# BradenDKelly/MetropolisMonteCarlo

Measured on AMD Instinct MI355X. Metric: MC trial moves/sec (whole node), SPC/E NVT full Ewald fp64, higher is better.
Workload: dtype f64

## Files before the change

metropolismontecarlo_amd/csrc/mmc_wave.hpp:

```cpp
#pragma once
#include "mmc_fast.hpp"
#include "mmc_propose.hpp"

#ifndef WV_WAVES
#define WV_WAVES 4
#endif
#ifndef WV_OCC
#define WV_OCC 5
#endif
#ifndef WV_OCC_WOLF
#define WV_OCC_WOLF 4
#endif
#ifndef WV_MWAVES
#define WV_MWAVES WV_WAVES
#endif
#ifndef WV_LIST
#define WV_LIST 640
#endif
#ifndef WV_PF
#define WV_PF 6
#endif
#define MMC_CQ_PAD (4 * 64 * (2 * WV_PF + 2))
#ifndef WV_TPF
#define WV_TPF 3
// ... 39 lines not shown
    __builtin_amdgcn_fence(__ATOMIC_ACQUIRE, "wavefront");
}

__device__ __forceinline__ double dpp_quad_swap_f64(double v)
{
    const long long b = __double_as_longlong(v);
    const unsigned lo = (unsigned)__builtin_amdgcn_update_dpp(0, (int)b, 0xB1, 0xf, 0xf, true),
                   hi = (unsigned)__builtin_amdgcn_update_dpp(0, (int)(b >> 32), 0xB1, 0xf, 0xf, true);
    return __longlong_as_double((long long)(((unsigned long long)hi << 32) | lo));
}
__device__ __forceinline__ void wave_sum6_add(double v0, double v1, double v2, double v3, double v4,
                                              double v5, double *out, double *scratch, int lane)
{
    const bool odd = (lane & 1) != 0;
    double p0 = (odd ? v1 : v0) + dpp_quad_swap_f64(odd ? v0 : v1);
    double p1 = (odd ? v3 : v2) + dpp_quad_swap_f64(odd ? v2 : v3);
    double p2 = (odd ? v5 : v4) + dpp_quad_swap_f64(odd ? v4 : v5);
    p0 += dpp_row_shr_f64<2>(p0); p1 += dpp_row_shr_f64<2>(p1); p2 += dpp_row_shr_f64<2>(p2);
    p0 += dpp_row_shr_f64<4>(p0); p1 += dpp_row_shr_f64<4>(p1); p2 += dpp_row_shr_f64<4>(p2);
    p0 += dpp_row_shr_f64<8>(p0); p1 += dpp_row_shr_f64<8>(p1); p2 += dpp_row_shr_f64<8>(p2);
    if ((lane & 14) == 14) {
        double *dst = scratch + 4 * (lane & 1) + (lane >> 4);
        dst[0] = p0; dst[8] = p1; dst[16] = p2;
    }
    __builtin_amdgcn_fence(__ATOMIC_RELEASE, "wavefront");
    __builtin_amdgcn_wave_barrier();
    __builtin_amdgcn_fence(__ATOMIC_ACQUIRE, "wavefront");
    if (lane < 6) {
        const double *r = scratch + 4 * lane;
        out[lane] += ((r[0] + r[1]) + r[2]) + r[3];
    }
}
__device__ __forceinline__ void wave_sum4_add(double v0, double v1, double v4, double v5, double *out,
                                              double *scratch, int lane)
{
    const bool odd = (lane & 1) != 0;
    double p0 = (odd ? v1 : v0) + dpp_quad_swap_f64(odd ? v0 : v1);
    double p1 = (odd ? v5 : v4) + dpp_quad_swap_f64(odd ? v4 : v5);
    p0 += dpp_row_shr_f64<2>(p0); p1 += dpp_row_shr_f64<2>(p1);
    p0 += dpp_row_shr_f64<4>(p0); p1 += dpp_row_shr_f64<4>(p1);
    p0 += dpp_row_shr_f64<8>(p0); p1 += dpp_row_shr_f64<8>(p1);
    if ((lane & 14) == 14) {
        double *dst = scratch + 4 * (lane & 1) + (lane >> 4);
        dst[0] = p0; dst[8] = p1;
    }
    __builtin_amdgcn_fence(__ATOMIC_RELEASE, "wavefront");
    __builtin_amdgcn_wave_barrier();
    __builtin_amdgcn_fence(__ATOMIC_ACQUIRE, "wavefront");
    if (lane < 4) {
        const double *r = scratch + 4 * lane;
        out[lane < 2 ? lane : lane + 2] += ((r[0] + r[1]) + r[2]) + r[3];
    }
}
__device__ __forceinline__ void wave_sum1_store(double v, double *out, double *scratch, int lane)
{
    v += dpp_row_shr_f64<1>(v);
    v += dpp_row_shr_f64<2>(v);
    v += dpp_row_shr_f64<4>(v);
    v += dpp_row_shr_f64<8>(v);
    if ((lane & 15) == 15)
        scratch[lane >> 4] = v;
    __builtin_amdgcn_fence(__ATOMIC_RELEASE, "wavefront");
    __builtin_amdgcn_wave_barrier();
    __builtin_amdgcn_fence(__ATOMIC_ACQUIRE, "wavefront");
    if (lane == 0)
        *out = ((scratch[0] + scratch[1]) + scratch[2]) + scratch[3];
}

__device__ __forceinline__ int lane_i32(int v, int src)
{
    return __builtin_amdgcn_readlane(v, src);
}

__device__ __forceinline__ double uniform_f64(double v)
{
    const long long b = __double_as_longlong(v);
    unsigned lo, hi;
    asm volatile("v_readfirstlane_b32 %0, %1" : "=s"(lo) : "v"((int)b));
    asm volatile("v_readfirstlane_b32 %0, %1" : "=s"(hi) : "v"((int)(b >> 32)));
    return __longlong_as_double((long long)(((unsigned long long)hi << 32) | lo));
}

__device__ __forceinline__ double lane_f64(double v, int src)
{
    const long long b = __double_as_longlong(v);
    const unsigned lo = (unsigned)__builtin_amdgcn_readlane((int)b, src);
    const unsigned hi = (unsigned)__builtin_amdgcn_readlane((int)(b >> 32), src);
    return __longlong_as_double((long long)(((unsigned long long)hi << 32) | lo));
}

__device__ __forceinline__ unsigned long long wave_shfl_xor_u64(unsigned long long v, int m)
{
    const unsigned lo = (unsigned)__shfl_xor((int)(unsigned)v, m, 64);
    const unsigned hi = (unsigned)__shfl_xor((int)(unsigned)(v >> 32), m, 64);
    return ((unsigned long long)hi << 32) | lo;
}
__device__ __forceinline__ unsigned long long wave_min_u64(unsigned long long v)
{
#pragma unroll
    for (int m = 32; m > 0; m >>= 1) {
        const unsigned long long o = wave_shfl_xor_u64(v, m);
        v = o < v ? o : v;
    }
    return v;
}

__device__ __forceinline__ void phase_row_moderate(double x, double L, cplx *row )
{
    double sn, cs;
    sincos_moderate(MMC_TWOPI * x / L, sn, cs);
    const cplx e1 = { cs, sn }, one = { 1.0, 0.0 };
    row[5] = one;
    row[6] = e1;
    row[4] = c_conj(e1);
    cplx p = e1;
#pragma unroll
    for (int k = 2; k <= 5; k++) {
        p = c_mul(p, e1);
        row[5 + k] = p;
        row[5 - k] = c_conj(p);
    }
}

__device__ __forceinline__ int wave_decide(const double *outw, bool ov_old, bool ov_new,
                                           const DecideConsts *__restrict__ dc, long long step, int r,
                                           int scur, int lane, double *delta_out = nullptr, bool store_flags = true,
                                           bool flip_s = true)
{
    const double delta = mmc_move_delta(outw, ov_old, ov_new, dc->factor);
    if (delta_out)
        *delta_out = delta;
    const double x = delta / dc->temperature;
    const double u = mmc_metropolis_uniform(ChainKey{ dc->seed, dc->replica0 + (uint32_t)r }, (uint64_t)step);
    bool met;
    if (x < 0.0) met = true;
    else if (1.0 - x > u + 1e-9) met = true;
    else if ((1.0 + x) * u > 1.0 + 1e-9) met = false;
    else met = exp(-x) > u;
    const int acc = (met && !(ov_old || ov_new)) ? 1 : 0;
    if (store_flags && lane == 0)
        dc->flags[r] = (uint8_t)(acc | ((scur ^ (flip_s ? acc : 0)) << 1));
    return acc;
}

__device__ __forceinline__ int wave_ticket(unsigned *queue, unsigned base, int n_waves, int lane)
{
    unsigned t = 0;
    if (lane == 0)
        t = atomicAdd(queue, 1u);
    return n_waves + (int)(__builtin_amdgcn_readfirstlane(t) - base);
}

template <bool SUBST, bool IMG, bool MULTI = false, bool WOLF = false>
__global__ __launch_bounds__(WV_MWAVES * 64)
__attribute__((amdgpu_waves_per_eu(WOLF ? WV_OCC_WOLF : WV_OCC, WOLF ? WV_OCC_WOLF : WV_OCC))) void k_move_eval_wave(
    BatchView bv, double *rec, const double *__restrict__ qq_tab,
    const int32_t *__restrict__ kpack, FastConsts fc, const MoveRec *__restrict__ cur,
    const MoveRec *__restrict__ prev, PartOut *out, int n_parts, PairParams pp, int r_base,
    int n_units, const uint8_t *flagv, unsigned stamp, const DecideConsts *__restrict__ dc, long long dec_step,
    int n_sub_arg, int slot0, unsigned *queue, unsigned queue_base)
{
    const int n_sub = MULTI ? n_sub_arg : 1;
    __shared__ __align__(16) WaveSharedT<WV_MWAVES, !WOLF> sm;
    const int tid = threadIdx.x, lane0 = tid & 63;
    const int wv = __builtin_amdgcn_readfirstlane(tid >> 6);

    for (int k = tid; k < MMC_QQ_TABLE_DOUBLES; k += WV_MWAVES * 64)
        sm.qtab[k] = qq_tab[k];
    __syncthreads();

    const int n_mol = bv.n_mol, nkv = bv.nkvecs;
    const double box = bv.box;
    const BoxConsts bc = box_consts(box);
    const int np = WOLF ? n_parts : (n_parts == 1) ? 1 : n_parts - 1;
    const int plen = (n_mol + np - 1) / np;
    const bool same_gate = pp.lj_gate_sq == pp.qq_gate_sq;
    const double inv_box = uniform_f64(1.0 / box);
    uint32_t gate_q;
    asm volatile("v_readfirstlane_b32 %0, %1" : "=s"(gate_q) : "v"(com_quant_gate(fmax(pp.lj_gate_sq, pp.qq_gate_sq), box)));
    wv_list_t *const list = sm.list[wv];
    const double *const pvw = sm.pvw[wv];

    for (int unit = blockIdx.x * WV_MWAVES + wv; unit < n_units;
         unit = MULTI && queue ? wave_ticket(queue, queue_base, gridDim.x * WV_MWAVES, lane0)
                               : unit + gridDim.x * WV_MWAVES) {
        int lane = lane0;
        if (!MULTI)
            asm volatile("" : "+v"(lane));
        int rl = unit, part = 0;
        if (n_parts != 1) {
            rl = unit / n_parts;
            part = unit - rl * n_parts;
        }
        const int r = r_base + rl;
        const bool do_pairs = WOLF ? true : (n_parts == 1) || (part < n_parts - 1);
        const bool do_recip = WOLF ? false : (n_parts == 1) || (part == n_parts - 1);
        const int j_begin = do_pairs ? min(part * plen, n_mol) : 0;
        const int j_end = do_pairs ? min(j_begin + plen, n_mol) : 0;
        double *const myrec = rec + (int64_t)r * n_mol * MMC_RSTRIDE;

        int flags_carry = -1;
        double e_sum = 0.0;
        unsigned acc_mask = 0, ovl_mask = 0, kind_mask = 0;
      for (int sub = 0; sub < n_sub; sub++) {
        if (MULTI) {
            lane = lane0;
            asm volatile("" : "+v"(lane));
        }
        const MoveRec *cur_s = cur, *prev_s = prev;
        if (n_sub > 1) {
            const int sl = (slot0 + sub) % dc->ring_slots, slp = (slot0 + sub + dc->ring_slots - 1) % dc->ring_slots;
            cur_s = dc->ring + (int64_t)sl * dc->ring_stride;
            if (sub > 0)
                prev_s = dc->ring + (int64_t)slp * dc->ring_stride;
        }
        WV_STAMP(0);
        const double *mvp = reinterpret_cast<const double *>(cur_s + r);
        double w = 0.0;
        if (lane < MV_Q_NEW)
            w = mvp[lane];
        WV_STAMP(1);
        const int gflag = flags_carry >= 0 ? flags_carry : (flagv ? __builtin_amdgcn_readfirstlane((int)flagv[r]) : -1);
        const long long hdr = __double_as_longlong(w);
        const int i0 = lane_i32((int)hdr, 0) - 1;
        const int flags = gflag >= 0 ? gflag : lane_i32((int)(hdr >> 32), 0);
        const bool commit = prev_s && (flags & 1);
        const int scur = (flags >> 1) & 1;

        int pend = -1;
        if (commit) {
            const double *pvp = reinterpret_cast<const double *>(prev_s + r);
            double pw = 0.0;
            if (lane < 9) pw = pvp[MV_AT_NEW + lane];
            else if (lane < 12) pw = pvp[MV_COM_NEW + lane - 9];
            else if (lane == 12) pw = pvp[0];
            else if (lane < 17) pw = pvp[MV_Q_NEW + lane - 13];
            pend = lane_i32((int)__double_as_longlong(pw), 12) - 1;
            if (lane < 12)
                sm.pvw[wv][lane] = pw;
            if (part == 0 && lane < 12) {
                myrec[(int64_t)pend * MMC_RSTRIDE + lane] = pw;
                if (lane < 9) {
                    const int a = lane / 3, d = lane % 3;
                    (d == 0 ? bv.ax : d == 1 ? bv.ay : bv.az)[r * bv.atom_stride + 3 * pend + a] = pw;
                } else {
                    const int d = lane - 9;
                    (d == 0 ? bv.comx : d == 1 ? bv.comy : bv.comz)[r * bv.mol_stride + pend] = pw;
                    comq_store(bv, r, pend, d, pw, inv_box);
                }
            }
            if (bv.quat) {
                const double q0 = wave_pick(pw, 13), q1 = wave_pick(pw, 14),
                             q2 = wave_pick(pw, 15), q3 = wave_pick(pw, 16);
                if (part == 0 && lane >= 13 && lane < 17)
                    quat_commit(bv, r, pend, lane - 13, pw, q0 * q0 + q1 * q1 + q2 * q2 + q3 * q3 > 0.25);
            }
            wave_sync();
            if (WOLF && !SUBST)
                asm volatile("s_waitcnt vmcnt(0)" ::: "memory");
        }

#define WV_CQ_BASE (bv.comq + (int64_t)r * 3 * bv.cq_stride)
#define WV_PART_DST (out + (int64_t)r * n_parts + part)
        auto decide_here = [&](bool o0, bool o1) -> int {
            if (!dc)
                return 0;
            if (n_sub <= 1)
                return wave_decide(sm.outw[wv], o0, o1, dc, dec_step, r, scur, lane, nullptr, true, !WOLF);
            double delta;
            const bool last = sub + 1 == n_sub;
            const int acc = wave_decide(sm.outw[wv], o0, o1, dc, dec_step + sub, r, scur, lane, &delta, last, !WOLF);
            if (acc) {
                e_sum += delta;
                acc_mask |= 1u << sub;
            }
            if (o0 || o1)
                ovl_mask |= 1u << sub;
            kind_mask |= (unsigned)((lane_i32((int)(hdr >> 32), 0) >> 8) & 1) << sub;
            flags_carry = acc | ((scur ^ (WOLF ? 0 : acc)) << 1);
            if (last) {
                wave_sync();
                if (lane < 7)
                    sm.outw[wv][lane] = lane == 0 ? e_sum
                                 : lane == 1 ? __longlong_as_double((long long)acc_mask | ((long long)ovl_mask << 32))
                                 : lane == 2 ? __longlong_as_double((long long)kind_mask) : 0.0;
                wave_sync();
            }
            return acc;
        };
#define WV_DECIDE(o0, o1) decide_here(o0, o1)
#define WV_RECORD_OVL(o) (n_sub > 1 ? false : (o))
#define WV_STORE_IF (sub + 1 == n_sub)
#define WV_STORE_SYSTEM MULTI
#define WV_ZERO opaque_f64(0.0)
#define WV_SUBST SUBST
#define WV_IMG IMG
#define WV_WOLF WOLF
#define WV_VIRIAL (!MULTI)
#ifndef WV_XY_MOVE
#define WV_XY_MOVE 1
#endif
#define WV_XY WV_XY_MOVE
#define WV_PASSES 2
#define WV_AFTER_PHASE_TABLES                                                                    \
    if (!SUBST && commit)                                                                        \
        asm volatile("s_waitcnt vmcnt(0)" ::: "memory");
#include "mmc_wave_unit.inc"
#undef WV_AFTER_PHASE_TABLES
#undef WV_IMG
#undef WV_WOLF
#undef WV_VIRIAL
#undef WV_PASSES
#undef WV_XY
#undef WV_SUBST
#undef WV_ZERO
#undef WV_CQ_BASE
#undef WV_PART_DST
#undef WV_DECIDE
#undef WV_RECORD_OVL
#undef WV_STORE_IF
#undef WV_STORE_SYSTEM
        if (n_sub > 1)
            asm volatile("s_waitcnt vmcnt(0)" ::: "memory");
      }
    }
}

struct TotalWaveShared {
    alignas(16) double qtab[MMC_QQ_TABLE_DOUBLES];
    int32_t list[WV_WAVES][WV_LIST];
};

#define WV_TOTAL_WAVES_PER_SIMD 5
template <bool COHERENT, bool IMG>
__device__ __forceinline__ void total_wave_body(
    TotalWaveShared &sm, const BatchView &bv, const double *__restrict__ rec,
    const double *__restrict__ qq_tab, const FastConsts &fc, const PairParams &pp, TotalPart *out,
    int units_per_rep, int n_units, int paired, int wg, int n_wgs, int j_chunk = 0)
{
    const int tid = threadIdx.x, lane0 = tid & 63;
    const int wv = __builtin_amdgcn_readfirstlane(tid >> 6);
    for (int k = tid; k < MMC_QQ_TABLE_DOUBLES; k += WV_WAVES * 64)
        sm.qtab[k] = qq_tab[k];
    __syncthreads();

    const int n_mol = bv.n_mol;
    const double box = bv.box;
    const BoxConsts bc = box_consts(box);
    const bool same_gate = pp.lj_gate_sq == pp.qq_gate_sq;
    const double inv_box = 1.0 / box;
    const uint32_t gate_q = com_quant_gate(fmax(pp.lj_gate_sq, pp.qq_gate_sq), box);
    int32_t *const list = sm.list[wv];

    for (int unit = wg * WV_WAVES + wv; unit < n_units; unit += n_wgs * WV_WAVES) {
        int lane = lane0;
        asm volatile("" : "+v"(lane));
        const int r = unit / units_per_rep, u = unit - r * units_per_rep;
        const double *myrec = rec + (int64_t)r * n_mol * MMC_RSTRIDE;
        const uint16_t *cq0 = bv.comq + (int64_t)r * 3 * bv.cq_stride;
        const uint32_t *sxy = reinterpret_cast<const uint32_t *>(cq0);
        const uint16_t *sz = cq0 + 2 * bv.cq_stride;
        double a_lj = 0, a_v = 0, a_q = 0;
        unsigned long long ovm = 0;

        const int n_ch = j_chunk > 0 ? (n_mol + j_chunk - 1) / j_chunk : 1;
        const int j_lo = j_chunk > 0 ? (u % n_ch) * j_chunk : 0;
        const int j_hi = j_chunk > 0 ? min(j_lo + j_chunk, n_mol) : n_mol;
        const int iA = j_chunk > 0 ? u / n_ch : u, iB = n_mol - 1 - u;
        const bool hasB = paired && iB > iA;
        double wAB = 0.0;
        if (lane < MMC_REC)
            wAB = myrec[(int64_t)iA * MMC_RSTRIDE + lane];
        else if (hasB && lane >= 16 && lane < 16 + MMC_REC)
            wAB = myrec[(int64_t)iB * MMC_RSTRIDE + lane - 16];

        auto process = [&](int cnt) {
            wave_sync();
            for (int n0 = 0; n0 < cnt; n0 += 64) {
                const int n = n0 + lane;
                const bool act = n < cnt;
                const int ent = act ? list[n] : 0;
                const int j = ent & ((1 << 27) - 1);
                const bool isB = (ent >> 27) != 0;
                double t[MMC_REC];
                const double2 *src = reinterpret_cast<const double2 *>(myrec + (int64_t)j * MMC_RSTRIDE);
#pragma unroll
                for (int q = 0; q < 6; q++) {
                    const double2 v = src[q];
                    t[2 * q] = v.x;
                    t[2 * q + 1] = v.y;
                }
                const int own0 = isB ? 16 : 0;
                auto mine = [&](int word) { return wave_pick(wAB, own0 + word); };
                const double ccx = mine(9), ccy = mine(10), ccz = mine(11);
                double m[3] = { 0, 0, 0 };
                auto min1 = [&](int d, double a, double b) {
                    if constexpr (IMG)
                        return fma(m[d], bc.neg, b - a);
                    else
                        return vector1D_abs(a, b, bc);
                };
                if constexpr (IMG) {
                    const double dx = t[9] - ccx, dy = t[10] - ccy, dz = t[11] - ccz;
                    m[0] = (fabs(dx) < bc.half) ? 0.0 : copysign(1.0, dx);
                    m[1] = (fabs(dy) < bc.half) ? 0.0 : copysign(1.0, dy);
                    m[2] = (fabs(dz) < bc.half) ? 0.0 : copysign(1.0, dz);
                }
                const double x0 = min1(0, ccx, t[9]), y0 = min1(1, ccy, t[10]), z0 = min1(2, ccz, t[11]);
                const double c0 = x0 * x0 + y0 * y0 + z0 * z0;
                const bool g0 = act && (c0 < pp.qq_gate_sq);
                const bool l0 = same_gate ? g0 : (act && (c0 < pp.lj_gate_sq));
                const unsigned long long gm0 = wave_ballot(g0);
                auto pair_ab = [&](int ab, double ax, double ay, double az, double bx, double by,
                                   double bz) {
                    const double qq = fc.qq9[ab];
                    const bool qneg = (fc.qneg_mask >> ab) & 1;
                    const double px = min1(0, ax, bx), py = min1(1, ay, by), pz = min1(2, az, bz);
                    const double u0 = px * px + py * py + pz * pz;
                    const unsigned long long cm0 = wave_ballot(u0 < pp.ovr) & gm0;
                    const unsigned long long im0 = (IMG ? ~0ULL : wave_ballot(u0 < pp.qq_slack_sq)) & (qneg ? gm0 & ~cm0 : gm0);
                    double e0 = qq_table_eval_lanes(sm.qtab, u0, im0);
                    if (qneg) {
                        ovm |= cm0;
                    } else if (cm0 != 0ULL) {
                        if (((im0 >> lane) & 1) && u0 < MMC_QQ_UMIN) e0 = qq_pair_cold(u0, pp.kappa);
                    }
                    a_q = fma(e0, qq, a_q);
                    const double eps = fc.eps9[ab], sg = fc.sig9[ab];
                    if ((fc.lj_mask >> ab) & 1) {
                        if (l0 && (IMG || u0 < pp.lj_slack_sq)) {
                            const double s2 = sg * sg / u0;
                            const double s6 = s2 * s2 * s2;
                            const double s12 = s6 * s6;
                            const double virab = eps * (2.0 * s12 - s6);
                            const double f0 = (IMG ? px : vector1D(ax, bx, bc)) * virab * s2,
                                         f1 = (IMG ? py : vector1D(ay, by, bc)) * virab * s2,
                                         f2 = (IMG ? pz : vector1D(az, bz, bc)) * virab * s2;
                            a_lj += eps * (s12 - s6);
                            a_v += (IMG ? x0 : vector1D(ccx, t[9], bc)) * f0 + (IMG ? y0 : vector1D(ccy, t[10], bc)) * f1
                                   + (IMG ? z0 : vector1D(ccz, t[11], bc)) * f2;
                        }
                    }
                };
#pragma unroll 1
                for (int a = 0; a < 3; a++) {
                    const double ax = mine(3 * a), ay = mine(3 * a + 1), az = mine(3 * a + 2);
                    pair_ab(3 * a, ax, ay, az, t[0], t[1], t[2]);
                    __builtin_amdgcn_sched_barrier(0);
                    pair_ab(3 * a + 1, ax, ay, az, t[3], t[4], t[5]);
                    __builtin_amdgcn_sched_barrier(0);
                    pair_ab(3 * a + 2, ax, ay, az, t[6], t[7], t[8]);
                    __builtin_amdgcn_sched_barrier(0);
                }
            }
            wave_sync();
        };

        int cnt = 0;
        for (int half = 0; half < (hasB ? 2 : 1); half++) {
            const int i0 = half == 0 ? iA : iB;
            const int woff = half == 0 ? 0 : 16;
            uint32_t cqxy, cqz;
            {
                const int t = lane & 15;
                const int myq = (t >= 9 && t < 12) ? (int)com_quant(wAB, inv_box) : 0;
                cqxy = (uint32_t)lane_i32(myq, woff + 9) | (uint32_t)lane_i32(myq, woff + 10) << 16;
                cqz = (uint32_t)lane_i32(myq, woff + 11);
            }
            const int first = max(i0 + 1, j_lo);
            int base = first & ~63;
            const char *pxy = reinterpret_cast<const char *>(sxy) + 4 * (int64_t)base;
            const char *pz = reinterpret_cast<const char *>(sz) + 2 * (int64_t)base;
            const uint32_t ul4 = 4u * (uint32_t)lane, ul2 = 2u * (uint32_t)lane;
            uint32_t fxy[WV_TPF], fz[WV_TPF];
#pragma unroll
            for (int b = 0; b < WV_TPF; b++) {
                fxy[b] = *reinterpret_cast<const uint32_t *>(pxy + 256 * b + ul4);
                fz[b] = *reinterpret_cast<const uint16_t *>(pz + 128 * b + ul2);
            }
            while (base < j_hi) {
#pragma unroll
                for (int b = 0; b < WV_TPF; b++) {
                    const int j = base + lane;
                    const uint32_t xy = fxy[b], z = fz[b];
                    fxy[b] = *reinterpret_cast<const uint32_t *>(pxy + 256 * (b + WV_TPF) + ul4);
                    fz[b] = *reinterpret_cast<const uint16_t *>(pz + 128 * (b + WV_TPF) + ul2);
                    const bool keep = (com_quant_dist2(xy, z, cqxy, cqz) < gate_q)
                                      && ((uint32_t)(j - first) < (uint32_t)(j_hi - first));
                    const unsigned long long m = wave_ballot(keep);
                    if (keep)
                        list[cnt + lanes_below(m)] = j | (half << 27);
                    cnt += __popcll(m);
                    base += 64;
                }
                pxy += 256 * WV_TPF;
                pz += 128 * WV_TPF;
                if (cnt > WV_LIST - 64 * WV_TPF) {
                    process(cnt);
                    cnt = 0;
                }
            }
        }
        if (cnt)
            process(cnt);
        const double s0 = wave_sum_rows(a_lj), s1 = wave_sum_rows(a_v), s2 = wave_sum_rows(a_q);
        const bool any_ovl = ovm != 0ULL;
        if (lane == 0) {
            TotalPart o;
            o.lj_pot = s0; o.lj_vir = s1; o.qq = s2;
            o.n_ovl = any_ovl ? 1 : 0;
            o._pad = 0;
            if (COHERENT) {
                double *w = reinterpret_cast<double *>(out + unit);
                __hip_atomic_store(w, o.lj_pot, __ATOMIC_RELAXED, __HIP_MEMORY_SCOPE_AGENT);
                __hip_atomic_store(w + 1, o.lj_vir, __ATOMIC_RELAXED, __HIP_MEMORY_SCOPE_AGENT);
                __hip_atomic_store(w + 2, o.qq, __ATOMIC_RELAXED, __HIP_MEMORY_SCOPE_AGENT);
                __hip_atomic_store(reinterpret_cast<long long *>(w + 3), (long long)o.n_ovl,
                                   __ATOMIC_RELAXED, __HIP_MEMORY_SCOPE_AGENT);
            } else {
                out[unit] = o;
            }
        }
    }
}

template <bool IMG>
__global__ __launch_bounds__(WV_WAVES * 64, WV_TOTAL_WAVES_PER_SIMD) void k_total_wave(
    BatchView bv, const double *__restrict__ rec, const double *__restrict__ qq_tab, FastConsts fc,
    PairParams pp, TotalPart *out, int units_per_rep, int n_units, int paired)
{
    __shared__ __align__(16) TotalWaveShared sm;
    total_wave_body<false, IMG>(sm, bv, rec, qq_tab, fc, pp, out, units_per_rep, n_units, paired,
                           (int)blockIdx.x, (int)gridDim.x);
}

__global__ __launch_bounds__(MMC_BLOCK) void k_total_reduce(const TotalPart *parts, int n_parts,
                                                             TotalsRaw *out)
{
    __shared__ double red[4 * MMC_WAVES];
    const int r = blockIdx.x;
    const TotalPart *p = parts + (int64_t)r * n_parts;
    double v[4] = { 0, 0, 0, 0 }, tot[4];
    for (int k = threadIdx.x; k < n_parts; k += MMC_BLOCK) {
        v[0] += p[k].lj_pot; v[1] += p[k].lj_vir; v[2] += p[k].qq; v[3] += (double)p[k].n_ovl;
    }
    block_sum<4>(v, red, tot);
    if (threadIdx.x == 0) {
        TotalsRaw t;
        t.lj_e = 2.0 * (tot[0] * 4);
        t.lj_v = 2.0 * (tot[1] * 24 / 3.0);
        t.qq = 2.0 * tot[2];
        t.n_ovl = tot[3] > 0 ? 1 : 0;
        t._pad = 0;
        out[r] = t;
    }
}

#define SRV_WAVES 8
struct ServerArgs {
    const unsigned long long *ctrl;
    const double2 *steps;
    uint64_t seed, replica0;
    int64_t rng_off;
    int32_t *timeout_flag;
    uint64_t seq_off;
};
#define SRV_ACCEPT 1u
#define SRV_SCUR 2u
#define SRV_STEPS 4u
#define SRV_QUIT 8u
#define SRV_TIMEOUT_TICKS 300000000ULL
#define SRV_GAVE_UP (~0ULL)

__global__ __launch_bounds__(SRV_WAVES * 64, 2) void k_move_server_wave(
    BatchView bv, double *rec, const double *__restrict__ qq_tab,
    const int32_t *__restrict__ kpack, FastConsts fc, PartOut *out, int n_parts, PairParams pp,
    ServerArgs sa)
{
    __shared__ __align__(16) WaveSharedT<SRV_WAVES> sm;
    __shared__ __align__(16) double mvw_all[SRV_WAVES][32];
    __shared__ __align__(16) double comb[8];
    __shared__ unsigned long long ctl;
    const int tid = threadIdx.x;
    int lane = tid & 63;
    const int wv = __builtin_amdgcn_readfirstlane(tid >> 6);
    for (int k = tid; k < MMC_QQ_TABLE_DOUBLES; k += blockDim.x)
        sm.qtab[k] = qq_tab[k];
    __syncthreads();

    const int n_mol = bv.n_mol, nkv = bv.nkvecs;
    const double box = bv.box;
    const BoxConsts bc = box_consts(box);
    const int np = n_parts - 1;
    const int plen = (n_mol + np - 1) / np;
    const bool same_gate = pp.lj_gate_sq == pp.qq_gate_sq;
    const double inv_box = 1.0 / box;
    const uint32_t gate_q = com_quant_gate(fmax(pp.lj_gate_sq, pp.qq_gate_sq), box);
    wv_list_t *const list = sm.list[wv];
    const double *const pvw = sm.pvw[wv];
    double *const mvw = mvw_all[wv];

    const int r = blockIdx.x, part = wv;
    const int unit = r * n_parts + part;
    (void)unit;
    const bool do_pairs = part < n_parts - 1;
    const bool do_recip = part == n_parts - 1;
    const int j_begin = do_pairs ? min(part * plen, n_mol) : 0;
    const int j_end = do_pairs ? min(j_begin + plen, n_mol) : 0;
    double *const myrec = rec + (int64_t)r * n_mol * MMC_RSTRIDE;
    const uint16_t *const cq_base = bv.comq + (int64_t)r * 3 * bv.cq_stride;
    PartOut *const part_dst = out + r;
    auto load_steps = [&]() {
        const double *p = reinterpret_cast<const double *>(sa.steps + r);
        return make_double2(__hip_atomic_load(p, __ATOMIC_RELAXED, __HIP_MEMORY_SCOPE_SYSTEM),
                            __hip_atomic_load(p + 1, __ATOMIC_RELAXED, __HIP_MEMORY_SCOPE_SYSTEM));
// ... 153 lines not shown
```

metropolismontecarlo_amd/csrc/mmc_wave_unit.inc:

```
#ifndef WV_NS
#define WV_NS 2
#define WV_NS_DEFAULTED
#endif
#if WV_NS == 2
#define WV_IF2(...) __VA_ARGS__
#else
#define WV_IF2(...)
#endif
#ifndef WV_SUBST
#define WV_SUBST 1
#define WV_SUBST_DEFAULTED
#endif
#ifndef WV_IMG
#define WV_IMG 0
#define WV_IMG_DEFAULTED
#endif
#ifndef WV_PASSES
#define WV_PASSES 1
#define WV_PASSES_DEFAULTED
#endif
#ifndef WV_XY
#define WV_XY 0
#define WV_XY_DEFAULTED
#endif
#ifndef WV_KPF
#define WV_KPF 2
#endif
#ifndef WV_WOLF
#define WV_WOLF 0
#define WV_WOLF_DEFAULTED
#endif
#ifndef WV_ZERO
#define WV_ZERO 0.0
#define WV_ZERO_DEFAULTED
#endif
#ifndef WV_VIRIAL
#define WV_VIRIAL 1
#define WV_VIRIAL_DEFAULTED
#endif
#ifndef WV_STORE_IF
#define WV_STORE_IF true
#define WV_STORE_IF_DEFAULTED
#endif
#if WV_NS != 2
static_assert(WV_VIRIAL, "the one-state body always delivers the virial");
#endif
        double *const outw = sm.outw[wv];
        unsigned long long ovm0 = 0, ovm1 = 0;

        constexpr bool wv_wolf = WV_WOLF;
        if constexpr (!wv_wolf) {
        if (do_recip) {
            {
                const int t = lane < 18 ? lane : 0;
                const int st = t / 9, q = t - 9 * st;
                const double x = wave_pick(w, (st ? MV_AT_NEW : MV_AT_OLD) + q);
                if (lane < 18)
                    phase_row_moderate(x, box, sm.ptab[wv][st][q / 3][q % 3]);
            }
            wave_sync();
            WV_STAMP(2);
#ifdef WV_AFTER_PHASE_TABLES
            WV_AFTER_PHASE_TABLES
#endif
        }
        auto recip_loop = [&]() {
            double a_rec = 0;
#ifdef WV_S_BASE
            const double *So = WV_S_BASE;
            double *Sn = WV_S_DST;
#else
            const double *So = s_buf(bv, r, scur);
            double *Sn = s_buf(bv, r, scur ^ 1);
#endif
            int kcs[WV_KPF], kps[WV_KPF];
            double cfs[WV_KPF];
            double2 sos[WV_KPF];
#pragma unroll
            for (int q = 0; q < WV_KPF; q++) {
                kcs[q] = min(lane + 64 * q, nkv - 1);
                kps[q] = kpack[kcs[q]];
                cfs[q] = bv.cfac[kcs[q]];
                sos[q] = *reinterpret_cast<const double2 *>(So + 2 * kcs[q]);
            }
#if WV_XY
            const int colp = kpack[MMC_NK_STRIDE + lane];
#endif
#if WV_XY
            cplx xyp[2][3];
            {
                const int cx = colp & 15, cy = (colp >> 4) & 15;
#pragma unroll
                for (int st = 0; st < 2; st++)
#pragma unroll
                    for (int l = 0; l < 3; l++)
                        xyp[st][l] = c_mul_fused(sm.ptab[wv][st][l][0][5 + cx], sm.ptab[wv][st][l][1][cy]);
            }
#endif
#ifdef WV_S_MIRROR
            unsigned long long s_sum = 0;
#endif
            const int n_it = (nkv + 63) >> 6;
            int k = lane;
            for (int it = 0; it < n_it; it++) {
                const int kc = kcs[0], kp = kps[0];
                const double cf = cfs[0];
                const double2 so = sos[0];
#pragma unroll
                for (int q = 0; q + 1 < WV_KPF; q++) {
                    kcs[q] = kcs[q + 1]; kps[q] = kps[q + 1]; cfs[q] = cfs[q + 1]; sos[q] = sos[q + 1];
                }
                kcs[WV_KPF - 1] = min(k + 64 * WV_KPF, nkv - 1);
                kps[WV_KPF - 1] = kpack[kcs[WV_KPF - 1]];
                cfs[WV_KPF - 1] = bv.cfac[kcs[WV_KPF - 1]];
                sos[WV_KPF - 1] = *reinterpret_cast<const double2 *>(So + 2 * kcs[WV_KPF - 1]);
                {
                    const int kz = (kp >> 8) & 15;
                    double nr = so.x, ni = so.y;
#if WV_XY
                    const int col = (kp >> 12) & (MMC_KCOLS - 1);
                    auto from_col = [&](const cplx &v) {
                        cplx o;
                        o.re = wave_pick(v.re, col);
                        o.im = wave_pick(v.im, col);
                        return o;
                    };
#else
                    const int kx = kp & 15, ky = (kp >> 4) & 15;
#endif
#pragma unroll
                    for (int l = 0; l < 3; l++) {
#if WV_XY
                        const cplx tn = c_mul_fused(from_col(xyp[1][l]), sm.ptab[wv][1][l][2][kz]);
                        const cplx to = c_mul_fused(from_col(xyp[0][l]), sm.ptab[wv][0][l][2][kz]);
#else
                        const cplx tn = c_mul_fused(c_mul_fused(sm.ptab[wv][1][l][0][5 + kx], sm.ptab[wv][1][l][1][ky]),
                                                sm.ptab[wv][1][l][2][kz]);
                        const cplx to = c_mul_fused(c_mul_fused(sm.ptab[wv][0][l][0][5 + kx], sm.ptab[wv][0][l][1][ky]),
                                                sm.ptab[wv][0][l][2][kz]);
#endif
                        nr = fma(fc.q[l], tn.re - to.re, nr);
                        ni = fma(fc.q[l], tn.im - to.im, ni);
                    }
                    *reinterpret_cast<double2 *>(Sn + 2 * kc) = make_double2(nr, ni);
#ifdef WV_S_MIRROR
                    {
                        typedef double s_piece __attribute__((ext_vector_type(2)));
                        s_piece v;
                        v.x = nr; v.y = ni;
                        double *mp = WV_S_MIRROR + 2 * kc;
                        asm volatile("global_store_dwordx4 %0, %1, off sc0 sc1" ::"v"(mp), "v"(v) : "memory");
                        if (k < nkv)
                            s_sum += (unsigned long long)__double_as_longlong(nr)
                                     + 3ULL * (unsigned long long)__double_as_longlong(ni);
                    }
#endif
                    const double wgt = k < nkv ? cf : 0.0;
                    a_rec = fma(wgt, fma(nr, nr, ni * ni) - fma(so.x, so.x, so.y * so.y), a_rec);
                }
                k += 64;
            }
            wave_sum1_store(a_rec, &outw[6], outw, lane);
#ifdef WV_S_MIRROR
            s_sum = wave_sum_u64(s_sum);
            if (lane == 0)
                sm.pvw[wv][0] = __longlong_as_double((long long)s_sum);
#endif
            WV_STAMP(3);
            wave_sync();
        };
        if (do_recip)
            recip_loop();
        }
        if (!do_recip && lane == 0)
            outw[6] = WV_ZERO;

        if (do_pairs) {
            if (lane < 6)
                outw[lane] = WV_ZERO;
            double cc[2][3];
            uint32_t cqxy[2], cqz[2];
            {
                const bool is_com = WV_IF2((lane >= MV_COM_OLD && lane < MV_COM_OLD + 3) ||)
                                    (lane >= MV_COM_NEW && lane < MV_COM_NEW + 3);
                const int myq = is_com ? (int)com_quant(w, inv_box) : 0;
#pragma unroll
                for (int d = 0; d < 3; d++) {
                    WV_IF2(cc[0][d] = lane_f64(w, MV_COM_OLD + d);)
                    cc[1][d] = lane_f64(w, MV_COM_NEW + d);
                }
                WV_IF2(cqxy[0] = (uint32_t)lane_i32(myq, MV_COM_OLD) | (uint32_t)lane_i32(myq, MV_COM_OLD + 1) << 16;)
                cqxy[1] = (uint32_t)lane_i32(myq, MV_COM_NEW) | (uint32_t)lane_i32(myq, MV_COM_NEW + 1) << 16;
                WV_IF2(cqz[0] = (uint32_t)lane_i32(myq, MV_COM_OLD + 2);)
                cqz[1] = (uint32_t)lane_i32(myq, MV_COM_NEW + 2);
            }

            auto process = [&](int cnt) {
                WV_IF2(double a_lj0 = 0, a_v0 = 0, a_q0 = 0;)
                double a_lj1 = 0, a_v1 = 0, a_q1 = 0;
                wave_sync();
                for (int n0 = 0; n0 < cnt; n0 += 64) {
                    const int n = n0 + lane;
                    const int j = n < cnt ? list[n] : 0;
                    const bool act = (n < cnt) && (j != i0);
                    double t[MMC_REC];
                    const double2 *src = reinterpret_cast<const double2 *>(myrec + (int64_t)j * MMC_RSTRIDE);
#pragma unroll
                    for (int q = 0; q < 6; q++) {
                        const double2 v = src[q];
                        t[2 * q] = v.x;
                        t[2 * q + 1] = v.y;
                    }
                    if (n0 == 0)
                        WV_STAMP(5);
                    if (WV_SUBST && j == pend) {
#pragma unroll
                        for (int q = 0; q < MMC_REC; q++)
                            t[q] = pvw[q];
                    }
                    WV_IF2(bool g0, l0;)
                    bool g1, l1;
                    constexpr bool wv_img = WV_IMG;
                    constexpr bool wv_virial = WV_VIRIAL;
                    double m[2][3] = { { 0, 0, 0 }, { 0, 0, 0 } };
                    auto min1 = [&](int st, int d, double a, double b) {
                        if constexpr (wv_img)
                            return fma(m[st][d], bc.neg, b - a);
                        else
                            return vector1D_abs(a, b, bc);
                    };
#define WV_MIN1(st, d, a, b) min1(st, d, a, b)
                    {
                        if constexpr (wv_img) {
#pragma unroll
                            for (int d = 0; d < 3; d++) {
                                const double d1 = t[9 + d] - cc[1][d];
                                m[1][d] = (fabs(d1) < bc.half) ? 0.0 : copysign(1.0, d1);
#if WV_NS == 2
                                const double d0 = t[9 + d] - cc[0][d];
                                m[0][d] = (fabs(d0) < bc.half) ? 0.0 : copysign(1.0, d0);
#endif
                            }
                        }
#if WV_NS == 2
                        const double x0 = WV_MIN1(0, 0, cc[0][0], t[9]), y0 = WV_MIN1(0, 1, cc[0][1], t[10]),
                                     z0 = WV_MIN1(0, 2, cc[0][2], t[11]);
                        const double c0 = x0 * x0 + y0 * y0 + z0 * z0;
                        g0 = act && (c0 < pp.qq_gate_sq);
                        l0 = same_gate ? g0 : (act && (c0 < pp.lj_gate_sq));
#endif
                        const double x1 = WV_MIN1(1, 0, cc[1][0], t[9]), y1 = WV_MIN1(1, 1, cc[1][1], t[10]),
                                     z1 = WV_MIN1(1, 2, cc[1][2], t[11]);
                        const double c1 = x1 * x1 + y1 * y1 + z1 * z1;
                        g1 = act && (c1 < pp.qq_gate_sq);
                        l1 = same_gate ? g1 : (act && (c1 < pp.lj_gate_sq));
                    }
                    WV_IF2(const unsigned long long gm0 = wave_ballot(g0);)
                    const unsigned long long gm1 = wave_ballot(g1);
#if WV_PASSES == 2
#define WV_PAIR_FENCE
                    auto pass = [&](auto stc, bool g, bool l, unsigned long long gm, unsigned long long &ovm,
                                    double &a_lj, double &a_v, double &a_q) {
                        constexpr int ST = decltype(stc)::value;
#pragma unroll 1
                        for (int a = 0; a < 3; a++) {
                            const int base_w = (ST ? MV_AT_NEW : MV_AT_OLD) + 3 * a;
                            const double ax = lane_f64(w, base_w), ay = lane_f64(w, base_w + 1),
                                         az = lane_f64(w, base_w + 2);
                            auto pair1 = [&](int ab, double bx, double by, double bz) {
                                const double qq = fc.qq9[ab];
                                const bool qneg = (fc.qneg_mask >> ab) & 1;
                                const double px = WV_MIN1(ST, 0, ax, bx), py = WV_MIN1(ST, 1, ay, by),
                                             pz = WV_MIN1(ST, 2, az, bz);
                                const double u = px * px + py * py + pz * pz;
                                const unsigned long long cm = wave_ballot(u < pp.ovr) & gm;
                                const unsigned long long qm = qneg ? cm : 0ULL, cold = cm & ~qm;
                                const unsigned long long im = (wv_img ? ~0ULL : wave_ballot(u < pp.qq_slack_sq)) & gm & ~qm;
                                double e = qq_table_eval_lanes(sm.qtab, u, im);
                                ovm |= qm;
                                if (cold != 0ULL) {
                                    if (((im >> lane) & 1) && u < MMC_QQ_UMIN) e = qq_pair_cold(u, pp.kappa);
                                }
                                a_q = fma(e, qq, a_q);
                                if ((fc.lj_mask >> ab) & 1) {
                                    const double eps = fc.eps9[ab], sg = fc.sig9[ab];
                                    if (l && (wv_img || u < pp.lj_slack_sq)) {
                                        const double s2 = sg * sg / u;
                                        const double s6 = s2 * s2 * s2;
                                        const double s12 = s6 * s6;
                                        double f0, f1, f2;
                                        if constexpr (wv_virial) {
                                            const double virab = eps * (2.0 * s12 - s6);
                                            f0 = (wv_img ? px : vector1D(ax, bx, bc)) * virab * s2;
                                            f1 = (wv_img ? py : vector1D(ay, by, bc)) * virab * s2;
                                            f2 = (wv_img ? pz : vector1D(az, bz, bc)) * virab * s2;
                                        }
                                        a_lj += eps * (s12 - s6);
                                        if constexpr (wv_virial) {
                                            a_v += (wv_img ? WV_MIN1(ST, 0, cc[ST][0], t[9]) : vector1D(cc[ST][0], t[9], bc)) * f0
                                                   + (wv_img ? WV_MIN1(ST, 1, cc[ST][1], t[10]) : vector1D(cc[ST][1], t[10], bc)) * f1
                                                   + (wv_img ? WV_MIN1(ST, 2, cc[ST][2], t[11]) : vector1D(cc[ST][2], t[11], bc)) * f2;
                                        }
                                    }
                                }
                            };
                            pair1(3 * a, t[0], t[1], t[2]);
                            WV_PAIR_FENCE
                            pair1(3 * a + 1, t[3], t[4], t[5]);
                            WV_PAIR_FENCE
                            pair1(3 * a + 2, t[6], t[7], t[8]);
                            WV_PAIR_FENCE
                        }
                        (void)g;
                    };
                    WV_IF2(pass(std::integral_constant<int, 0>{}, g0, l0, gm0, ovm0, a_lj0, a_v0, a_q0);)
                    pass(std::integral_constant<int, 1>{}, g1, l1, gm1, ovm1, a_lj1, a_v1, a_q1);
                }
#else
                    auto pair_ab = [&](int ab, double a0x, double a0y, double a0z, double a1x,
                                       double a1y, double a1z, double bx, double by, double bz) {
                        const double qq = fc.qq9[ab];
                        const bool qneg = (fc.qneg_mask >> ab) & 1;
#if WV_NS == 2
                        const double p0x = WV_MIN1(0, 0, a0x, bx), p0y = WV_MIN1(0, 1, a0y, by),
                                     p0z = WV_MIN1(0, 2, a0z, bz);
                        const double u0 = p0x * p0x + p0y * p0y + p0z * p0z;
                        const unsigned long long cm0 = wave_ballot(u0 < pp.ovr) & gm0;
                        const unsigned long long im0 = wave_ballot(u0 < pp.qq_slack_sq) & (qneg ? gm0 & ~cm0 : gm0);
                        double e0 = qq_table_eval_lanes(sm.qtab, u0, im0);
#else
                        (void)a0x; (void)a0y; (void)a0z;
#endif
                        const double p1x = WV_MIN1(1, 0, a1x, bx), p1y = WV_MIN1(1, 1, a1y, by),
                                     p1z = WV_MIN1(1, 2, a1z, bz);
                        const double u1 = p1x * p1x + p1y * p1y + p1z * p1z;
                        const unsigned long long cm1 = wave_ballot(u1 < pp.ovr) & gm1;
                        const unsigned long long im1 = wave_ballot(u1 < pp.qq_slack_sq) & (qneg ? gm1 & ~cm1 : gm1);
                        double e1 = qq_table_eval_lanes(sm.qtab, u1, im1);
                        if (qneg) {
                            WV_IF2(ovm0 |= cm0;)
                            ovm1 |= cm1;
                        } else if ((WV_IF2(cm0 |) cm1) != 0ULL) {
                            WV_IF2(if (((im0 >> lane) & 1) && u0 < MMC_QQ_UMIN) e0 = qq_pair_cold(u0, pp.kappa);)
                            if (((im1 >> lane) & 1) && u1 < MMC_QQ_UMIN) e1 = qq_pair_cold(u1, pp.kappa);
                        }
                        WV_IF2(a_q0 = fma(e0, qq, a_q0);)
                        a_q1 = fma(e1, qq, a_q1);
                        const double eps = fc.eps9[ab], sg = fc.sig9[ab];
                        if ((fc.lj_mask >> ab) & 1) {
#if WV_NS == 2
                            if (l0 && u0 < pp.lj_slack_sq) {
                                const double s2 = sg * sg / u0;
                                const double s6 = s2 * s2 * s2;
                                const double s12 = s6 * s6;
                                double f0, f1, f2;
                                if constexpr (wv_virial) {
                                    const double virab = eps * (2.0 * s12 - s6);
                                    f0 = (wv_img ? p0x : vector1D(a0x, bx, bc)) * virab * s2;
                                    f1 = (wv_img ? p0y : vector1D(a0y, by, bc)) * virab * s2;
                                    f2 = (wv_img ? p0z : vector1D(a0z, bz, bc)) * virab * s2;
                                }
                                a_lj0 += eps * (s12 - s6);
                                if constexpr (wv_virial) {
                                    a_v0 += (wv_img ? WV_MIN1(0, 0, cc[0][0], t[9]) : vector1D(cc[0][0], t[9], bc)) * f0
                                            + (wv_img ? WV_MIN1(0, 1, cc[0][1], t[10]) : vector1D(cc[0][1], t[10], bc)) * f1
                                            + (wv_img ? WV_MIN1(0, 2, cc[0][2], t[11]) : vector1D(cc[0][2], t[11], bc)) * f2;
                                }
                            }
#endif
                            if (l1 && u1 < pp.lj_slack_sq) {
                                const double s2 = sg * sg / u1;
                                const double s6 = s2 * s2 * s2;
                                const double s12 = s6 * s6;
                                double f0, f1, f2;
                                if constexpr (wv_virial) {
                                    const double virab = eps * (2.0 * s12 - s6);
                                    f0 = (wv_img ? p1x : vector1D(a1x, bx, bc)) * virab * s2;
                                    f1 = (wv_img ? p1y : vector1D(a1y, by, bc)) * virab * s2;
                                    f2 = (wv_img ? p1z : vector1D(a1z, bz, bc)) * virab * s2;
                                }
                                a_lj1 += eps * (s12 - s6);
                                if constexpr (wv_virial) {
                                    a_v1 += (wv_img ? WV_MIN1(1, 0, cc[1][0], t[9]) : vector1D(cc[1][0], t[9], bc)) * f0
                                            + (wv_img ? WV_MIN1(1, 1, cc[1][1], t[10]) : vector1D(cc[1][1], t[10], bc)) * f1
                                            + (wv_img ? WV_MIN1(1, 2, cc[1][2], t[11]) : vector1D(cc[1][2], t[11], bc)) * f2;
                                }
                            }
                        }
                    };
#pragma unroll 1
                    for (int a = 0; a < 3; a++) {
#if WV_NS == 2
                        const double a0x = lane_f64(w, MV_AT_OLD + 3 * a),
                                     a0y = lane_f64(w, MV_AT_OLD + 3 * a + 1),
                                     a0z = lane_f64(w, MV_AT_OLD + 3 * a + 2);
#else
                        const double a0x = 0.0, a0y = 0.0, a0z = 0.0;
#endif
                        const double a1x = lane_f64(w, MV_AT_NEW + 3 * a),
                                     a1y = lane_f64(w, MV_AT_NEW + 3 * a + 1),
                                     a1z = lane_f64(w, MV_AT_NEW + 3 * a + 2);
                        pair_ab(3 * a, a0x, a0y, a0z, a1x, a1y, a1z, t[0], t[1], t[2]);
                        __builtin_amdgcn_sched_barrier(0);
                        pair_ab(3 * a + 1, a0x, a0y, a0z, a1x, a1y, a1z, t[3], t[4], t[5]);
                        __builtin_amdgcn_sched_barrier(0);
                        pair_ab(3 * a + 2, a0x, a0y, a0z, a1x, a1y, a1z, t[6], t[7], t[8]);
                        __builtin_amdgcn_sched_barrier(0);
                    }
                }
#endif
#undef WV_MIN1
#if WV_NS == 2
                if constexpr (WV_VIRIAL)
                    wave_sum6_add(a_lj0, a_lj1, a_v0, a_v1, a_q0, a_q1, outw, sm.sum6w(wv), lane);
                else
                    wave_sum4_add(a_lj0, a_lj1, a_q0, a_q1, outw, sm.sum6w(wv), lane);
#else
                const double s1 = wave_sum_rows(a_lj1), s3 = wave_sum_rows(a_v1), s5 = wave_sum_rows(a_q1);
                if (lane == 0) {
                    outw[1] += s1; outw[3] += s3; outw[5] += s5;
                }
#endif
                wave_sync();
            };

            const char *pxy = reinterpret_cast<const char *>(WV_CQ_BASE) + 4 * (int64_t)j_begin;
            const char *pz = reinterpret_cast<const char *>(WV_CQ_BASE + 2 * bv.cq_stride) + 2 * (int64_t)j_begin;
            const uint32_t ul4 = 4u * (uint32_t)lane, ul2 = 2u * (uint32_t)lane;
            uint32_t pqxy = 0, pqz = 0;
            if (WV_SUBST && pend >= 0) {
                pqxy = (uint32_t)__builtin_amdgcn_readfirstlane((int)com_quant(pvw[9], inv_box))
                       | (uint32_t)__builtin_amdgcn_readfirstlane((int)com_quant(pvw[10], inv_box)) << 16;
                pqz = (uint32_t)__builtin_amdgcn_readfirstlane((int)com_quant(pvw[11], inv_box));
            }
            int base = j_begin, cnt = 0;
            uint32_t fxy[WV_PF], fz[WV_PF];
#pragma unroll
            for (int b = 0; b < WV_PF; b++) {
                fxy[b] = *reinterpret_cast<const uint32_t *>(pxy + 256 * b + ul4);
                fz[b] = *reinterpret_cast<const uint16_t *>(pz + 128 * b + ul2);
            }
            while (base < j_end) {
#pragma unroll
                for (int b = 0; b < WV_PF; b++) {
                    const int j = base + lane;
                    uint32_t xy = fxy[b], z = fz[b];
                    fxy[b] = *reinterpret_cast<const uint32_t *>(pxy + 256 * (b + WV_PF) + ul4);
                    fz[b] = *reinterpret_cast<const uint16_t *>(pz + 128 * (b + WV_PF) + ul2);
                    if (WV_SUBST && j == pend) { xy = pqxy; z = pqz; }
                    const bool keep = WV_IF2((com_quant_dist2(xy, z, cqxy[0], cqz[0]) < gate_q) |)
                                      (com_quant_dist2(xy, z, cqxy[1], cqz[1]) < gate_q);
                    const int nv = j_end - base;
                    const unsigned long long m_end = nv >= 64 ? ~0ULL : (nv > 0 ? (1ULL << nv) - 1ULL : 0ULL);
                    const unsigned long long m = wave_ballot(keep);
                    if (keep)
                        list[cnt + lanes_below(m)] = j;
                    cnt += __popcll(m & m_end);
                    base += 64;
                }
                pxy += 256 * WV_PF;
                pz += 128 * WV_PF;
                if (cnt > WV_LIST - 64 * WV_PF) {
                    process(cnt);
                    cnt = 0;
                }
            }
            WV_STAMP(4);
            if (cnt)
                process(cnt);
            WV_STAMP(6);
        } else if (lane < 6) {
            outw[lane] = WV_ZERO;
        }
#ifdef WV_S_MIRROR
        if (do_recip && !do_pairs) {
            wave_sync();
            if (lane == 0)
                outw[0] = sm.pvw[wv][0];
        }
#endif

#ifdef WV_UNIT_NO_STORE
        if (lane == 0)
            outw[7] = __longlong_as_double((long long)((ovm0 != 0ULL ? 1 : 0) | (ovm1 != 0ULL ? 2 : 0)));
#else
        wave_sync();
        {
#ifdef WV_DECIDE
            const int accept = WV_DECIDE(ovm0 != 0ULL, ovm1 != 0ULL);
#else
            const int accept = 0;
#endif
            if (WV_STORE_IF) {
                const uint32_t csum = part_checksum_lanes(lane < 7 ? outw[lane] : 0.0, lane, stamp);
#ifdef WV_RECORD_OVL
                if (lane == 0)
                    outw[7] = pack_ovl(WV_RECORD_OVL(ovm0 != 0ULL), WV_RECORD_OVL(ovm1 != 0ULL), stamp, csum, accept);
#else
                if (lane == 0)
                    outw[7] = pack_ovl(ovm0 != 0ULL, ovm1 != 0ULL, stamp, csum, accept);
#endif
            }
        }
        wave_sync();
#ifdef WV_STORE_WT
        store_part<true>(WV_PART_DST, sm.outw[wv], lane);
#else
#ifndef WV_STORE_SYSTEM
#define WV_STORE_SYSTEM false
#define WV_STORE_SYSTEM_DEFAULTED
#endif
        if (WV_STORE_IF)
            store_part<WV_STORE_SYSTEM>(WV_PART_DST, sm.outw[wv], lane);
#ifdef WV_STORE_SYSTEM_DEFAULTED
#undef WV_STORE_SYSTEM
#undef WV_STORE_SYSTEM_DEFAULTED
#endif
#endif
        wave_sync();
        WV_STAMP(7);
#endif
#ifdef WV_STORE_IF_DEFAULTED
#undef WV_STORE_IF
#undef WV_STORE_IF_DEFAULTED
#endif
#undef WV_IF2
#ifdef WV_XY_DEFAULTED
#undef WV_XY
#undef WV_XY_DEFAULTED
#endif
#ifdef WV_PASSES_DEFAULTED
#undef WV_PASSES
#undef WV_PASSES_DEFAULTED
#endif
#ifdef WV_IMG_DEFAULTED
#undef WV_IMG
#undef WV_IMG_DEFAULTED
#endif
#ifdef WV_SUBST_DEFAULTED
#undef WV_SUBST
#undef WV_SUBST_DEFAULTED
#endif
#ifdef WV_ZERO_DEFAULTED
#undef WV_ZERO
#undef WV_ZERO_DEFAULTED
#endif
#ifdef WV_VIRIAL_DEFAULTED
#undef WV_VIRIAL
#undef WV_VIRIAL_DEFAULTED
#endif
#ifdef WV_WOLF_DEFAULTED
#undef WV_WOLF
#undef WV_WOLF_DEFAULTED
#endif
#ifdef WV_NS_DEFAULTED
#undef WV_NS
#undef WV_NS_DEFAULTED
#endif
```

Baseline: 151.3 million.

## Add fast-path pair pass with rare exact overlap recheck and single process call site

The two-pass pair loop now first runs a fast variant that skips the overlap and cold-table ballots. It tracks the minimum squared distance through the high 32 bits of the double, and reruns the exact path only when any gated lane falls below the overlap threshold. The neighbour-list build loop is also restructured so process() has a single call site, re-priming the prefetch buffers after each flush. This cuts per-pair ballots and code size, but can do the work twice in rare overlap cases and adds a refetch at each list flush.

```diff
diff --git a/metropolismontecarlo_amd/csrc/mmc_wave.hpp b/metropolismontecarlo_amd/csrc/mmc_wave.hpp
--- a/metropolismontecarlo_amd/csrc/mmc_wave.hpp
+++ b/metropolismontecarlo_amd/csrc/mmc_wave.hpp
@@ -365,6 +365,10 @@
 #endif
 #define WV_XY WV_XY_MOVE
 #define WV_PASSES 2
+#ifndef WV_ONE_CALL_MOVE
+#define WV_ONE_CALL_MOVE 1
+#endif
+#define WV_ONE_CALL WV_ONE_CALL_MOVE
 #define WV_AFTER_PHASE_TABLES                                                                    \
     if (!SUBST && commit)                                                                        \
         asm volatile("s_waitcnt vmcnt(0)" ::: "memory");
@@ -374,6 +378,7 @@
 #undef WV_WOLF
 #undef WV_VIRIAL
 #undef WV_PASSES
+#undef WV_ONE_CALL
 #undef WV_XY
 #undef WV_SUBST
 #undef WV_ZERO
diff --git a/metropolismontecarlo_amd/csrc/mmc_wave_unit.inc b/metropolismontecarlo_amd/csrc/mmc_wave_unit.inc
--- a/metropolismontecarlo_amd/csrc/mmc_wave_unit.inc
+++ b/metropolismontecarlo_amd/csrc/mmc_wave_unit.inc
@@ -18,6 +18,10 @@
 #ifndef WV_PASSES
 #define WV_PASSES 1
 #define WV_PASSES_DEFAULTED
+#endif
+#ifndef WV_ONE_CALL
+#define WV_ONE_CALL 0
+#define WV_ONE_CALL_DEFAULTED
 #endif
 #ifndef WV_XY
 #define WV_XY 0
@@ -259,9 +263,11 @@
                     const unsigned long long gm1 = wave_ballot(g1);
 #if WV_PASSES == 2
 #define WV_PAIR_FENCE
-                    auto pass = [&](auto stc, bool g, bool l, unsigned long long gm, unsigned long long &ovm,
+                    auto pass = [&](auto stc, bool l, unsigned long long gm, unsigned long long &ovm,
                                     double &a_lj, double &a_v, double &a_q) {
                         constexpr int ST = decltype(stc)::value;
+                        auto atoms = [&](auto exc, uint32_t &umin) {
+                        constexpr bool EXACT = decltype(exc)::value;
 #pragma unroll 1
                         for (int a = 0; a < 3; a++) {
                             const int base_w = (ST ? MV_AT_NEW : MV_AT_OLD) + 3 * a;
@@ -269,19 +275,26 @@
                                          az = lane_f64(w, base_w + 2);
                             auto pair1 = [&](int ab, double bx, double by, double bz) {
                                 const double qq = fc.qq9[ab];
-                                const bool qneg = (fc.qneg_mask >> ab) & 1;
                                 const double px = WV_MIN1(ST, 0, ax, bx), py = WV_MIN1(ST, 1, ay, by),
                                              pz = WV_MIN1(ST, 2, az, bz);
                                 const double u = px * px + py * py + pz * pz;
-                                const unsigned long long cm = wave_ballot(u < pp.ovr) & gm;
-                                const unsigned long long qm = qneg ? cm : 0ULL, cold = cm & ~qm;
-                                const unsigned long long im = (wv_img ? ~0ULL : wave_ballot(u < pp.qq_slack_sq)) & gm & ~qm;
-                                double e = qq_table_eval_lanes(sm.qtab, u, im);
-                                ovm |= qm;
-                                if (cold != 0ULL) {
-                                    if (((im >> lane) & 1) && u < MMC_QQ_UMIN) e = qq_pair_cold(u, pp.kappa);
-                                }
+                                const unsigned long long km = (wv_img ? ~0ULL : wave_ballot(u < pp.qq_slack_sq)) & gm;
+                                if constexpr (EXACT) {
+                                    const bool qneg = (fc.qneg_mask >> ab) & 1;
+                                    const unsigned long long cm = wave_ballot(u < pp.ovr) & gm;
+                                    const unsigned long long qm = qneg ? cm : 0ULL, cold = cm & ~qm;
+                                    const unsigned long long im = km & ~qm;
+                                    double e = qq_table_eval_lanes(sm.qtab, u, im);
+                                    ovm |= qm;
+                                    if (cold != 0ULL) {
+                                        if (((im >> lane) & 1) && u < MMC_QQ_UMIN) e = qq_pair_cold(u, pp.kappa);
+                                    }
+                                    a_q = fma(e, qq, a_q);
+                                } else {
+                                umin = min(umin, (uint32_t)(__double_as_longlong(u) >> 32));
+                                const double e = qq_table_eval_lanes(sm.qtab, u, km);
                                 a_q = fma(e, qq, a_q);
+                                asm volatile("" : "+v"(a_q));
                                 if ((fc.lj_mask >> ab) & 1) {
                                     const double eps = fc.eps9[ab], sg = fc.sig9[ab];
                                     if (l && (wv_img || u < pp.lj_slack_sq)) {
@@ -303,6 +316,7 @@
                                         }
                                     }
                                 }
+                                }
                             };
                             pair1(3 * a, t[0], t[1], t[2]);
                             WV_PAIR_FENCE
@@ -311,10 +325,18 @@
                             pair1(3 * a + 2, t[6], t[7], t[8]);
                             WV_PAIR_FENCE
                         }
-                        (void)g;
+                        };
+                        const double a_q_in = a_q;
+                        uint32_t umin = ~0u;
+                        atoms(std::false_type{}, umin);
+                        const uint32_t thr_hi = (uint32_t)(__double_as_longlong(pp.ovr) >> 32);
+                        if (__builtin_expect((wave_ballot(umin <= thr_hi) & gm) != 0ULL, 0)) {
+                            a_q = a_q_in;
+                            atoms(std::true_type{}, umin);
+                        }
                     };
-                    WV_IF2(pass(std::integral_constant<int, 0>{}, g0, l0, gm0, ovm0, a_lj0, a_v0, a_q0);)
-                    pass(std::integral_constant<int, 1>{}, g1, l1, gm1, ovm1, a_lj1, a_v1, a_q1);
+                    WV_IF2(pass(std::integral_constant<int, 0>{}, l0, gm0, ovm0, a_lj0, a_v0, a_q0);)
+                    pass(std::integral_constant<int, 1>{}, l1, gm1, ovm1, a_lj1, a_v1, a_q1);
                 }
 #else
                     auto pair_ab = [&](int ab, double a0x, double a0y, double a0z, double a1x,
@@ -435,12 +457,20 @@
             }
             int base = j_begin, cnt = 0;
             uint32_t fxy[WV_PF], fz[WV_PF];
+#if WV_ONE_CALL
+            while (base < j_end) {
+            cnt = 0;
+#endif
 #pragma unroll
             for (int b = 0; b < WV_PF; b++) {
                 fxy[b] = *reinterpret_cast<const uint32_t *>(pxy + 256 * b + ul4);
                 fz[b] = *reinterpret_cast<const uint16_t *>(pz + 128 * b + ul2);
             }
+#if WV_ONE_CALL
+            while (base < j_end && cnt <= WV_LIST - 64 * WV_PF) {
+#else
             while (base < j_end) {
+#endif
 #pragma unroll
                 for (int b = 0; b < WV_PF; b++) {
                     const int j = base + lane;
@@ -460,6 +490,13 @@
                 }
                 pxy += 256 * WV_PF;
                 pz += 128 * WV_PF;
+#if WV_ONE_CALL
+            }
+            WV_STAMP(4);
+            if (cnt)
+                process(cnt);
+            }
+#else
                 if (cnt > WV_LIST - 64 * WV_PF) {
                     process(cnt);
                     cnt = 0;
@@ -468,6 +505,7 @@
             WV_STAMP(4);
             if (cnt)
                 process(cnt);
+#endif
             WV_STAMP(6);
         } else if (lane < 6) {
             outw[lane] = WV_ZERO;
@@ -529,6 +567,10 @@
 #undef WV_XY
 #undef WV_XY_DEFAULTED
 #endif
+#ifdef WV_ONE_CALL_DEFAULTED
+#undef WV_ONE_CALL
+#undef WV_ONE_CALL_DEFAULTED
+#endif
 #ifdef WV_PASSES_DEFAULTED
 #undef WV_PASSES
 #undef WV_PASSES_DEFAULTED
```

New measurement: 155.3 million (median of 6 runs). 1.03x the previous value.
